# versatiles-org/versatiles-glyphs-rs

Measured on AMD Instinct MI355X. Metric: glyphs/sec (SDF raster, Noto Sans Regular full BMP set), higher is better.
Workload: dtype f64

## Files before the change

versatiles-glyphs-rs_amd/csrc/sdf_margin_kernels.hip:

```cpp
#include <hip/hip_runtime.h>
#include <stdint.h>

#include "sdf_span_support.h"

#ifndef VG_MARGIN_PART
#error "compile with -DVG_MARGIN_PART=0..6"
#endif
#define VG_MARGIN_PARTS 7
#define VG_CAT_(a, b) a##b
#define VG_CAT(a, b) VG_CAT_(a, b)

namespace vgsdf {

typedef void (*span_fn)(const GlyphDesc *, const uint2 *, uint32_t, const double *, const double *, const double *, const double *,
                        uint32_t, uint8_t *, const float4 *, const PlanHeader *);
struct MarginInstance {
	int id;
	span_fn fn;
};

#if VG_MARGIN_PART == 0
#define VG_SPAN_KERNEL sdf_margin_span_base
#include "sdf_span_kernel.inc"
__device__ unsigned long long g_span_dbg[28];
#define VG_SPAN_KERNEL sdf_margin_span_count
#define VG_SPAN_COUNTED 1
#define VG_COUNT(stmt) stmt
#include "sdf_span_kernel.inc"
#undef VG_SPAN_COUNTED
#define VG_SPAN_KERNEL sdf_margin_span_dl0
#define VG_M_DL(dl) ((void)(dl), 0.0f)
#define VG_M_E8(e, f1) ((void)(e), (void)(f1), true)
#include "sdf_span_kernel.inc"
#define VG_SPAN_KERNEL sdf_margin_span_e0
#define VG_M_E(e) ((void)(e), 0.0f)
#define VG_M_E64(e) ((void)(e), 0.0f)
#include "sdf_span_kernel.inc"
static const MarginInstance k_instances[] = {{60, sdf_margin_span_base}, {61, sdf_margin_span_count}, {62, sdf_margin_span_dl0}, {63, sdf_margin_span_e0}};

#elif VG_MARGIN_PART == 1
#define VG_SPAN_KERNEL sdf_margin_span_tkf1
#define VG_M_TK(tk, f1) ((void)(tk), (f1))
#include "sdf_span_kernel.inc"
#define VG_SPAN_KERNEL sdf_margin_span_rg0
#define VG_M_RG(r) ((void)(r), 0.0f)
#include "sdf_span_kernel.inc"
#define VG_SPAN_KERNEL sdf_margin_span_sat3
#define VG_M_SAT 3.0f
#include "sdf_span_kernel.inc"
#define VG_SPAN_KERNEL sdf_margin_span_far20
#define VG_M_FAR 20.0f
#include "sdf_span_kernel.inc"
static const MarginInstance k_instances[] = {{64, sdf_margin_span_tkf1}, {65, sdf_margin_span_rg0}, {66, sdf_margin_span_sat3}, {67, sdf_margin_span_far20}};

#elif VG_MARGIN_PART == 2
#define VG_SPAN_KERNEL sdf_margin_span_sane
#define VG_M_SANE(Mc) ((void)(Mc), true)
#include "sdf_span_kernel.inc"
#define VG_SPAN_KERNEL sdf_margin_span_bounded
#define VG_M_BOUNDED(Mc) ((void)(Mc), true)
#include "sdf_span_kernel.inc"
#define VG_SPAN_KERNEL sdf_margin_span_boxr0
#define VG_M_BOX_R(r) ((void)(r), 0.0f)
#include "sdf_span_kernel.inc"
#define VG_SPAN_KERNEL sdf_margin_span_boxband
#define VG_M_BOX_BAND(dy) ((void)(dy), true)
#include "sdf_span_kernel.inc"
static const MarginInstance k_instances[] = {{68, sdf_margin_span_sane}, {69, sdf_margin_span_bounded}, {70, sdf_margin_span_boxr0}, {71, sdf_margin_span_boxband}};

#elif VG_MARGIN_PART == 3
#define VG_SPAN_KERNEL sdf_margin_span_e64
#define VG_M_E64(e) ((void)(e), 0.0f)
#include "sdf_span_kernel.inc"
#define VG_SPAN_KERNEL sdf_margin_span_mabs0
#define VG_M_MABS0(m) ((void)(m), 0.0f)
#include "sdf_span_kernel.inc"
#define VG_SPAN_KERNEL sdf_margin_span_infl
#define VG_M_INFL 1.0f
#define VG_M_PAD(Mc) ((void)(Mc), 0.0f)
#define VG_M_GRP_SLACK 1.0f
#include "sdf_span_kernel.inc"
#define VG_SPAN_KERNEL sdf_margin_span_e_2
#define VG_M_E(e) ((e) * 0.5f)
#include "sdf_span_kernel.inc"
static const MarginInstance k_instances[] = {{72, sdf_margin_span_e64}, {73, sdf_margin_span_mabs0}, {74, sdf_margin_span_infl}, {75, sdf_margin_span_e_2}};

#elif VG_MARGIN_PART == 4
#define VG_SPAN_KERNEL sdf_margin_span_e_4
#define VG_M_E(e) ((e) * 0.25f)
#include "sdf_span_kernel.inc"
#define VG_SPAN_KERNEL sdf_margin_span_e_8
#define VG_M_E(e) ((e) * 0.125f)
#include "sdf_span_kernel.inc"
#define VG_SPAN_KERNEL sdf_margin_span_dl_2
#define VG_M_DL(dl) ((dl) * 0.5f)
#include "sdf_span_kernel.inc"
#define VG_SPAN_KERNEL sdf_margin_span_dl_4
#define VG_M_DL(dl) ((dl) * 0.25f)
#include "sdf_span_kernel.inc"
static const MarginInstance k_instances[] = {{76, sdf_margin_span_e_4}, {77, sdf_margin_span_e_8}, {78, sdf_margin_span_dl_2}, {79, sdf_margin_span_dl_4}};

#elif VG_MARGIN_PART == 5
#define VG_SPAN_KERNEL sdf_margin_span_dl_8
#define VG_M_DL(dl) ((dl) * 0.125f)
#include "sdf_span_kernel.inc"
#define VG_SPAN_KERNEL sdf_margin_span_rg_2
#define VG_M_RG(r) ((r) * 0.5f)
#include "sdf_span_kernel.inc"
#define VG_SPAN_KERNEL sdf_margin_span_rg_4
#define VG_M_RG(r) ((r) * 0.25f)
#include "sdf_span_kernel.inc"
#define VG_SPAN_KERNEL sdf_margin_span_rg_8
#define VG_M_RG(r) ((r) * 0.125f)
#include "sdf_span_kernel.inc"
static const MarginInstance k_instances[] = {{80, sdf_margin_span_dl_8}, {81, sdf_margin_span_rg_2}, {82, sdf_margin_span_rg_4}, {83, sdf_margin_span_rg_8}};
#elif VG_MARGIN_PART == 6
#define VG_SPAN_KERNEL sdf_margin_span_row_e0
#define VG_M_ROW_E(e) ((void)(e), 0.0f)
#include "sdf_span_kernel.inc"
static const MarginInstance k_instances[] = {{84, sdf_margin_span_row_e0}};

#else
#error "VG_MARGIN_PART out of range"
#endif

}

extern "C" __attribute__((visibility("hidden"))) int VG_CAT(vgsdf_margin_launch_p, VG_MARGIN_PART)(
    int kernel, uint32_t grid, uint32_t n_tiles_arg, const vgsdf::GlyphDesc *glyphs, const uint2 *tiles, const double *sx, const double *sy,
    const double *ex, const double *ey, uint32_t seg_stride, uint8_t *out, const void *boxes, hipStream_t stream)
{
	for (const vgsdf::MarginInstance &m : vgsdf::k_instances)
		if (m.id == kernel) {
			hipLaunchKernelGGL(m.fn, dim3(grid), dim3(vgsdf::TPB), 0, stream, glyphs, tiles, n_tiles_arg, sx, sy, ex, ey, seg_stride, out,
			                   (const float4 *)boxes, (const vgsdf::PlanHeader *)nullptr);
			return (int)hipGetLastError();
		}
	return -1;
}

#if VG_MARGIN_PART == 0
#define VG_MARGIN_PART_ARGS                                                                                                          \
	int kernel, uint32_t grid, uint32_t n_tiles_arg, const vgsdf::GlyphDesc *glyphs, const uint2 *tiles, const double *sx, const double *sy, \
	    const double *ex, const double *ey, uint32_t seg_stride, uint8_t *out, const void *boxes, hipStream_t stream
extern "C" int vgsdf_margin_launch_p1(VG_MARGIN_PART_ARGS);
extern "C" int vgsdf_margin_launch_p2(VG_MARGIN_PART_ARGS);
extern "C" int vgsdf_margin_launch_p3(VG_MARGIN_PART_ARGS);
extern "C" int vgsdf_margin_launch_p4(VG_MARGIN_PART_ARGS);
extern "C" int vgsdf_margin_launch_p5(VG_MARGIN_PART_ARGS);
extern "C" int vgsdf_margin_launch_p6(VG_MARGIN_PART_ARGS);

extern "C" int vgsdf_margin_known(int kernel) { return kernel >= 60 && kernel <= 84; }

extern "C" int vgsdf_margin_launch(VG_MARGIN_PART_ARGS)
{
	int (*const parts[VG_MARGIN_PARTS])(VG_MARGIN_PART_ARGS) = {vgsdf_margin_launch_p0, vgsdf_margin_launch_p1, vgsdf_margin_launch_p2,
	                                                            vgsdf_margin_launch_p3, vgsdf_margin_launch_p4, vgsdf_margin_launch_p5,
	                                                            vgsdf_margin_launch_p6};
	for (auto part : parts) {
		const int e = part(kernel, grid, n_tiles_arg, glyphs, tiles, sx, sy, ex, ey, seg_stride, out, boxes, stream);
		if (e != -1)
			return e;
	}
	return (int)hipErrorInvalidValue;
}

extern "C" int vgsdf_margin_counters(unsigned long long *out, int reset)
{
	unsigned long long h[28] = {0};
	hipError_t e = hipSuccess;
	if (out != nullptr) {
		e = hipMemcpyFromSymbol(h, HIP_SYMBOL(vgsdf::g_span_dbg), sizeof(h), 0, hipMemcpyDeviceToHost);
		static const int idx[9] = {12, 13, 14, 15, 16, 17, 20, 21, 22};
		for (int i = 0; i < 9; i++)
			out[i] = h[idx[i]];
	}
	if (e == hipSuccess && reset) {
		const unsigned long long z[28] = {0};
		e = hipMemcpyToSymbol(HIP_SYMBOL(vgsdf::g_span_dbg), z, sizeof(z), 0, hipMemcpyHostToDevice);
	}
	return (int)e;
}

extern "C" int vgsdf_margin_pair_round_counters(unsigned long long *out)
{
	unsigned long long h[28] = {0};
	const hipError_t e = hipMemcpyFromSymbol(h, HIP_SYMBOL(vgsdf::g_span_dbg), sizeof(h), 0, hipMemcpyDeviceToHost);
	for (int i = 0; i < 2; i++)
		out[i] = h[23 + i];
	return (int)e;
}

extern "C" int vgsdf_margin_stage_filter_counters(unsigned long long *out)
{
	unsigned long long h[28] = {0};
	const hipError_t e = hipMemcpyFromSymbol(h, HIP_SYMBOL(vgsdf::g_span_dbg), sizeof(h), 0, hipMemcpyDeviceToHost);
	out[0] = h[25];
	return (int)e;
}
#endif
```

versatiles-glyphs-rs_amd/csrc/sdf_span_kernel.inc:

```
#ifndef VG_POOL_MAX
#define VG_POOL_MAX 2
#endif
#ifndef VG_SPAN_KERNEL
#define VG_SPAN_KERNEL sdf_tiles_span
#endif
#ifndef VG_STAMP
#define VG_STAMP(region)
#endif
#ifndef VG_COUNT
#define VG_COUNT(stmt)
#endif
#ifndef VG_M_BOX_PADK
#define VG_M_BOX_PADK(mag) (0.02f + 2.0e-6f * (mag))
#endif
#ifndef VG_M_BOX_SAT
#define VG_M_BOX_SAT 6.2f
#endif
#ifndef VG_M_BOX_R
#define VG_M_BOX_R(r) (r)
#endif
#ifndef VG_M_BOX_BAND
#define VG_M_BOX_BAND(dy) ((dy) > 0.0f)
#endif
#ifndef VG_M_INFL
#define VG_M_INFL (1.0f + 1.0f / 512.0f)
#endif
#ifndef VG_M_GRP_SLACK
#define VG_M_GRP_SLACK 1.004f
#endif
#ifndef VG_M_PAD
#define VG_M_PAD(Mc) (0.01f + 1.0e-5f * (Mc))
#endif
#ifndef VG_M_RG
#define VG_M_RG(r) (r)
#endif
#ifndef VG_M_SAT
#define VG_M_SAT 6.2f
#endif
#ifndef VG_M_SANE
#define VG_M_SANE(Mc) ((Mc) < 1.0e6f)
#endif
#ifndef VG_M_BOUNDED
#define VG_M_BOUNDED(Mc) ((Mc) < 4096.0f)
#endif
#ifndef VG_M_MABS0
#define VG_M_MABS0(m) (m)
#endif
#ifndef VG_M_E64
#define VG_M_E64(e) (e)
#endif
#ifndef VG_M_E
#define VG_M_E(e) (e)
#endif
#ifndef VG_M_CARRY
#define VG_M_CARRY (1.0f + 1.0f / 1048576.0f)
#endif
#ifndef VG_M_DL
#define VG_M_DL(dl) (dl)
#endif
#ifndef VG_M_DL_C
#define VG_M_DL_C 17.0f
#endif
#ifndef VG_M_DL_ABS
#define VG_M_DL_ABS 3.0e-4f
#endif
#ifndef VG_M_E8
#define VG_M_E8(e, f1) (8.0f * (e) <= (f1))
#endif
#ifndef VG_M_FAR
#define VG_M_FAR 35.9f
#endif
#ifndef VG_M_TK_PUSH
#define VG_M_TK_PUSH(tk) ((tk) * 1.001f + 1e-30f)
#endif
#ifndef VG_M_TK
#define VG_M_TK(tk, f1) (tk)
#endif
#ifndef VG_M_ROW_E
#define VG_M_ROW_E(e) (e)
#endif

__global__ __launch_bounds__(TPB, 4) void VG_SPAN_KERNEL(const GlyphDesc *__restrict__ glyphs,
                                                          const uint2 *__restrict__ tiles, uint32_t n_tiles,
                                                          const double *__restrict__ seg_sx,
                                                          const double *__restrict__ seg_sy,
                                                          const double *__restrict__ seg_ex,
                                                          const double *__restrict__ seg_ey, uint32_t seg_stride,
                                                          uint8_t *__restrict__ out, const float4 *__restrict__ boxes,
                                                          const PlanHeader *__restrict__ plan)
{
	if (plan != nullptr && (!plan->ok || blockIdx.x >= plan->n_main))
		return;
#ifdef VG_SPAN_STAMPED
	unsigned long long st_acc[12] = {0, 0, 0, 0, 0, 0, 0, 0, 0, 0, 0, 0}, st_last = 0;
#endif
#if defined(VG_SPAN_STAMPED) || defined(VG_SPAN_COUNTED)
	unsigned long long cn_pairs = 0, cn_rounds = 0, cn_tc = 0, cn_fb = 0, cn_fbl = 0;
	unsigned long long cn_over = 0, cn_fb_pool = 0, cn_fb_lane = 0;
	unsigned long long cn_half = 0, cn_leave = 0;
	unsigned long long cn_row_fb = 0;
#endif
	VG_STAMP(-1);
	constexpr uint32_t GRP = 8, NGRP = FCHUNK / GRP;
	static_assert(NGRP == 32 && TPB == FCHUNK, "one candidate bit per group, one staging thread per record");
	__shared__ __attribute__((aligned(16))) float s_rec[5][FCHUNK];
	__shared__ double e_pt[4][FCHUNK];
	float *const s_vx = s_rec[0], *const s_vy = s_rec[1], *const s_dx = s_rec[2], *const s_dy = s_rec[3], *const s_inv = s_rec[4];
	double *const e_vx = e_pt[0], *const e_vy = e_pt[1], *const e_wx = e_pt[2], *const e_wy = e_pt[3];
	__shared__ int s_delta[DELTA_CAP];
	__shared__ uint32_t s_mbits[2];
	__shared__ __attribute__((aligned(16))) float s_g[3][NGRP];
	__shared__ float st_ub2[SPAN_TILES * TPB];
	__shared__ uint16_t st_byte[SPAN_TILES * TPB];
	__shared__ uint32_t st_pix[SPAN_TILES * TPB];
	constexpr uint32_t QCAP = 256;
	__shared__ uint32_t q_pair[TPB / 64][QCAP];
	__shared__ uint32_t q_min[TPB / 64][64];

	const uint32_t tid = threadIdx.x, lane = threadIdx.x & 63;
	const uint32_t wv = (uint32_t)__builtin_amdgcn_readfirstlane((int)(threadIdx.x >> 6));
	const uint32_t rot = wave_rot(blockIdx.x);
	const uint32_t pw = ((wv + rot) & 3u) * 64u;
	const uint32_t tile = xcd_remap(blockIdx.x, n_tiles);
	const uint2 t = tiles[tile];
	const GlyphDesc g = glyphs[t.x];
	const uint32_t npix = g.w * g.h;
	const uint32_t p0 = t.y & ~255u, T = min(max(t.y & 255u, 1u), SPAN_TILES);
	const uint32_t p_end = min(p0 + T * (uint32_t)TPB, npix);

	const uint32_t r_first = p0 / g.w, r_last = (p_end - 1) / g.w;
	const int y_hi = (int)(g.h - 1 - r_first), y_lo = (int)(g.h - 1 - r_last);
	const uint32_t stride = (g.w + 1) | 1u;
	const uint32_t n_delta = (r_last - r_first + 1) * stride;
	for (uint32_t i = tid; i < n_delta; i += TPB)
		s_delta[i] = 0;
	const float wh = (float)max(g.w, g.h);
	const int hw = (int)(g.w >> 1), hh = (int)(g.h >> 1);
	for (uint32_t k = 0; k < T; k++) {
		st_ub2[k * TPB + tid] = __builtin_inff();
		st_byte[k * TPB + tid] = 0x00FFu;
		const uint32_t oc = min(p0 + k * TPB + pw + lane, npix - 1);
		const uint32_t row = oc / g.w;
		st_pix[k * TPB + tid] = pix_pack((float)((int)(oc - row * g.w) - hw) + 0.5f, row - r_first);
	}
	int y_mid = y_hi - hh;
	asm volatile("" : "+s"(y_mid));
	const float mpix = 0.5f * wh + 1.0f;
	uint32_t par = 0;
	if (tid == 0)
		s_mbits[0] = __float_as_uint(mpix);
	const float mabs0 = VG_M_MABS0(fmaxf(fmaxf(fabsf((float)g.x0), fabsf((float)g.y0)),
	                                     fmaxf(fabsf((float)g.x0 + (float)g.w), fabsf((float)g.y0 + (float)g.h))));

	const bool use_boxes = boxes != nullptr && g.n_seg > 2 * FCHUNK;
	for (uint32_t c0 = 0; c0 < g.n_seg; c0 += FCHUNK) {
		const uint32_t cnt = min((uint32_t)FCHUNK, g.n_seg - c0);
		VG_STAMP(0);
		__syncthreads();
		VG_STAMP(1);
		if (use_boxes) {
			const float4 bb = boxes[chunk_box_index(g.seg_off, t.x, c0 / FCHUNK)];
			const float mag = fmaxf(fmaxf(fabsf(bb.x), fabsf(bb.y)), fmaxf(fmaxf(fabsf(bb.z), fabsf(bb.w)), wh));
			const float padk = VG_M_BOX_PADK(mag);
			const float ry0 = (float)y_lo + 0.5f, ry1 = (float)y_hi + 0.5f;
			const float dy = fmaxf(bb.y - ry1, ry0 - bb.w) - padk;
			float dx = fmaxf(bb.x - ((float)g.w - 0.5f), 0.5f - bb.z) - padk;
			dx = dx > 0.0f ? dx : 0.0f;
			const float R = VG_M_BOX_R(VG_M_BOX_SAT + padk);
			if (VG_M_BOX_BAND(dy) && __builtin_fmaf(dy, dy, dx * dx) > R * R)
				continue;
		}
		constexpr float INFL = VG_M_INFL;
		{
			int gx0 = g.x0, gy0 = g.y0;
			asm volatile("" : "+s"(gx0), "+s"(gy0));
			const double ox = (double)gx0 + (double)hw, oy = (double)gy0 + (double)hh;
			const uint32_t i = tid;
			float mf = 0.0f;
			float fvx = 1.0e18f, fvy = 1.0e18f, fdx = 0.0f, fdy = 0.0f, finv = 0.0f;
			uint32_t nrow = 0;
			int ya = 0;
			bool row_exact = false;
			if (i < cnt) {
				const size_t s = (size_t)(g.seg_off + c0 + i) * seg_stride;
				const double vx = seg_sx[s], vy = seg_sy[s], wx = seg_ex[s], wy = seg_ey[s];
				e_vx[i] = vx;
				e_vy[i] = vy;
				e_wx[i] = wx;
				e_wy[i] = wy;
				const double dx = wx - vx, dy = wy - vy;
				const double l2 = dx * dx + dy * dy;
				fvx = (float)(vx - ox);
				fvy = (float)(vy - oy);
				fdx = (float)dx;
				fdy = (float)dy;
				finv = (l2 > 1e-20 && l2 < 1e30) ? __builtin_amdgcn_rcpf((float)l2) : 0.0f;
				mf = fmaxf(fmaxf(fabsf(fvx), fabsf(fvy)), fmaxf(fabsf(fvx + fdx), fabsf(fvy + fdy))) * 1.00001f;
				mf = mf >= 0.0f ? mf : __builtin_inff();
				const float tv = fvy - 0.5f, tw = (fvy + fdy) - 0.5f;
				const float e_row = VG_M_ROW_E(__builtin_fmaf(STAGE_ROW_C, fmaxf(mf, mpix), STAGE_ROW_ABS));
				const bool decided = __builtin_fminf(int_dist(tv), int_dist(tw)) > e_row && mf < STAGE_M_MAX;
				const int cv = (int)__builtin_ceilf(tv), cw = (int)__builtin_ceilf(tw);
				const int c_lo = y_lo - hh, c_hi = y_hi + 1 - hh;
				const int ca = min(max(min(cv, cw), c_lo), c_hi), cb = min(max(max(cv, cw), c_lo), c_hi);
				ya = ca + hh;
				nrow = decided ? (uint32_t)(cb - ca) : 0u;
				row_exact = vy != wy && !decided;
			}
			const bool row_fb = __builtin_amdgcn_ballot_w64(row_exact) != 0;
			VG_COUNT(cn_row_fb += row_fb);
			if (row_fb && row_exact) {
				const double vy = e_vy[i], wy = e_wy[i];
				const double y0c = (double)gy0 + 0.5;
				const double band_lo = (double)y_lo + y0c, band_hi = (double)y_hi + y0c;
				const bool up = vy < wy;
				const double lo = up ? vy : wy, hi = up ? wy : vy;
				if (hi > band_lo && lo <= band_hi) {
					ya = first_ge(lo, y0c, y_lo, y_hi + 1);
					const int yb = first_ge(hi, y0c, y_lo, y_hi + 1);
					nrow = yb > ya ? (uint32_t)(yb - ya) : 0u;
				}
			}
			s_vx[i] = fvx;
			s_vy[i] = fvy;
			s_dx[i] = fdx;
			s_dy[i] = fdy;
			s_inv[i] = finv;
			const uint32_t mb = wave_max_u32(__float_as_uint(mf));
			if (lane == 0)
				atomicMax(&s_mbits[par], mb);

			{
				const uint32_t gb = tid & ~(GRP - 1);
				const uint32_t ai = min(gb + GRP / 2, cnt - 1);
				const float ax = __shfl(fvx, (int)(ai & 63u)), ay = __shfl(fvy, (int)(ai & 63u));
				float r2 = 0.0f;
				if (i < cnt) {
					const float wx = fvx + fdx, wy = fvy + fdy;
					const float ex = fvx - ax, ey = fvy - ay, fx = wx - ax, fy = wy - ay;
					const float dv = __builtin_fmaf(ey, ey, ex * ex), dw = __builtin_fmaf(fy, fy, fx * fx);
					r2 = dv > dw ? dv : dw;
				}
				r2 = __uint_as_float(oct_max_u32(__float_as_uint(r2)));
				if ((tid & (GRP - 1)) == 0) {
					const bool empty = gb >= cnt;
					s_g[0][tid / GRP] = empty ? 1.0e18f : ax;
					s_g[1][tid / GRP] = empty ? 1.0e18f : ay;
					s_g[2][tid / GRP] = empty ? 0.0f : __builtin_amdgcn_sqrtf(r2) * (INFL * INFL * VG_M_GRP_SLACK);
				}
			}

			{
				const uint32_t incl = wave_scan_add(nrow);
				const uint32_t total = (uint32_t)__builtin_amdgcn_readlane((int)incl, 63);
				auto cross = [&](double vx, double vy, double dx, double dy, bool up, int yy) {
					const double x0c = (double)gx0 + 0.5, y0c = (double)gy0 + 0.5;
					const double pyy = (double)yy + y0c;
					const double tc = (pyy - vy) / dy;
					const double xc = vx + tc * dx;
					const int k = first_ge(xc, x0c, 0, (int)g.w);
					if (k < (int)g.w)
						atomicAdd(&s_delta[(uint32_t)(y_hi - yy) * stride + (uint32_t)k], up ? -1 : 1);
				};
				if (total != 0 && total <= QCAP) {
					uint32_t off = incl - nrow;
#pragma unroll 1
					for (uint32_t r = 0; r < nrow; r++)
						q_pair[wv][off++] = (lane << 10) | (uint32_t)(y_hi - (ya + (int)r));
					__builtin_amdgcn_fence(__ATOMIC_RELEASE, "wavefront");
					__builtin_amdgcn_wave_barrier();
					for (uint32_t base = 0; base < total; base += 64) {
						const uint32_t idx = base + lane;
						if (idx < total) {
							const uint32_t e = q_pair[wv][idx];
							const uint32_t si = (tid & ~63u) + (e >> 10);
							const double vx = e_vx[si], vy = e_vy[si], wx = e_wx[si], wy = e_wy[si];
							cross(vx, vy, wx - vx, wy - vy, vy < wy, y_hi - (int)(e & 1023u));
						}
					}
					__builtin_amdgcn_fence(__ATOMIC_ACQ_REL, "wavefront");
					__builtin_amdgcn_wave_barrier();
				} else if (total != 0) {
					if (nrow != 0) {
						const double vx = e_vx[i], vy = e_vy[i], wx = e_wx[i], wy = e_wy[i];
						for (uint32_t r = 0; r < nrow; r++)
							cross(vx, vy, wx - vx, wy - vy, vy < wy, ya + (int)r);
					}
				}
			}
		}
		VG_STAMP(2);
		__syncthreads();
		VG_STAMP(3);
		const float Mc = __uint_as_float(s_mbits[par]);
		par ^= 1u;
		if (tid == 0)
			s_mbits[par] = __float_as_uint(mpix);
		const bool sane = VG_M_SANE(Mc);
		const bool bounded = VG_M_BOUNDED(Mc);
		const float pad = VG_M_PAD(Mc);
		const uint32_t n_groups = (cnt + GRP - 1) / GRP;

		const float4 *q_vx = reinterpret_cast<const float4 *>(s_vx), *q_vy = reinterpret_cast<const float4 *>(s_vy);
		const float4 *q_dx = reinterpret_cast<const float4 *>(s_dx), *q_dy = reinterpret_cast<const float4 *>(s_dy);
		const float4 *q_inv = reinterpret_cast<const float4 *>(s_inv);
		const float M = Mc;
		const float e64 = VG_M_E64(VG_E64_C * M * (M + mabs0 + M));
		const float herr_c1 = VG_HERR_SLACK * VG_HERR_C1 * M, herr_c3 = VG_HERR_SLACK * VG_HERR_C3 * M * M + e64;

#pragma unroll 1
		for (uint32_t k = 0; k < T; k++) {
			asm volatile("" ::: "memory");
			const uint32_t o = p0 + k * TPB + pw + lane;
			if (p0 + k * TPB + pw >= npix)
				continue;
			const uint32_t pe = st_pix[k * TPB + tid];
			const float rpx = pix_rpx(pe);
			const int roff = (int)pix_roff(pe);
			const float rpy = (float)(y_mid - roff) + 0.5f;
			float ub2 = st_ub2[k * TPB + tid];
			VG_STAMP(0);


			uint32_t cand = n_groups >= 32 ? 0xFFFFFFFFu : ((1u << n_groups) - 1u);
			if (bounded) {
				uint32_t D2p[NGRP / 2];
				uint32_t dmin = __float_as_uint(ub2);
				const float4 *gx4 = reinterpret_cast<const float4 *>(s_g[0]), *gy4 = reinterpret_cast<const float4 *>(s_g[1]);
				const float4 *gr4 = reinterpret_cast<const float4 *>(s_g[2]);
				auto near4 = [&](uint32_t b, const float4 ax, const float4 ay) {
					const float axs[4] = {ax.x, ax.y, ax.z, ax.w}, ays[4] = {ay.x, ay.y, ay.z, ay.w};
					uint32_t d2[4];
#pragma unroll
					for (int j = 0; j < 4; j++) {
						const float ddx = rpx - axs[j], ddy = rpy - ays[j];
						d2[j] = __float_as_uint(__builtin_fmaf(ddy, ddy, ddx * ddx));
					}
					asm("v_min3_u32 %0, %1, %2, %3" : "=v"(dmin) : "v"(dmin), "v"(d2[0]), "v"(d2[1]));
					asm("v_min3_u32 %0, %1, %2, %3" : "=v"(dmin) : "v"(dmin), "v"(d2[2]), "v"(d2[3]));
					D2p[b * 2] = __builtin_amdgcn_perm(d2[1], d2[0], 0x07060302u);
					D2p[b * 2 + 1] = __builtin_amdgcn_perm(d2[3], d2[2], 0x07060302u);
				};
				if (n_groups == NGRP) {
#pragma unroll
					for (uint32_t b = 0; b < NGRP / 4; b++)
						near4(b, gx4[b], gy4[b]);
				} else {
					float4 ax = gx4[0], ay = gy4[0];
#pragma unroll
					for (uint32_t b = 0; b < NGRP / 4; b++) {
						if (b * 4 < n_groups) {
							if (b + 1 == NGRP / 4) {
								near4(b, ax, ay);
								break;
							}
							const float4 nx = gx4[b + 1], ny = gy4[b + 1];
							near4(b, ax, ay);
							asm volatile("" ::"v"(nx.x), "v"(nx.y), "v"(nx.z), "v"(nx.w), "v"(ny.x), "v"(ny.y), "v"(ny.z), "v"(ny.w));
							ax = nx;
							ay = ny;
						} else {
							break;
						}
					}
				}
				ub2 = __uint_as_float(dmin);
				float U = (__builtin_amdgcn_sqrtf(ub2) * INFL + pad) * INFL;
				U = U < VG_M_SAT ? U : VG_M_SAT;
				const float Ui = (U + pad * INFL) * VG_M_GRP_SLACK;
				uint32_t rej;
				asm volatile("" : "=v"(rej));
				auto reject4 = [&](uint32_t b) {
					const float4 r = gr4[b];
					const float rs[4] = {r.x, r.y, r.z, r.w};
#pragma unroll
					for (int j = 3; j >= 0; j--) {
						const uint32_t pk = D2p[b * 2 + j / 2];
						const float d2 = __uint_as_float((j & 1) ? pk : (pk << 16));
						const float tt = Ui + VG_M_RG(rs[j]);
						const float diff = __builtin_fmaf(tt, tt, -d2);
						rej = __builtin_amdgcn_alignbit(rej, __float_as_uint(diff), 31);
					}
				};
				static_assert(NGRP / 4 == 8, "one case per block of four groups");
				if (n_groups == NGRP) {
#pragma unroll
					for (int b = NGRP / 4 - 1; b >= 0; b--)
						reject4((uint32_t)b);
				} else switch ((n_groups + 3) / 4) {
				default: reject4(7); [[fallthrough]];
				case 7: reject4(6); [[fallthrough]];
				case 6: reject4(5); [[fallthrough]];
				case 5: reject4(4); [[fallthrough]];
				case 4: reject4(3); [[fallthrough]];
				case 3: reject4(2); [[fallthrough]];
				case 2: reject4(1); [[fallthrough]];
				case 1: reject4(0);
				}
				cand &= ~rej;
			}

			VG_STAMP(6);
			uint32_t k1 = 0xFFFFFFFFu;
			auto rec4 = [](const float4 *row, uint32_t goff, uint32_t hq) {
				return *reinterpret_cast<const float4 *>(reinterpret_cast<const char *>(row) + goff + 16u * hq);
			};
			auto half_min = [&](uint32_t acc, uint32_t goff, uint32_t hq, float qx, float qy) {
				const float4 vx4 = rec4(q_vx, goff, hq), vy4 = rec4(q_vy, goff, hq), dx4 = rec4(q_dx, goff, hq), dy4 = rec4(q_dy, goff, hq),
				             iv4 = rec4(q_inv, goff, hq);
				const uint32_t f0 = __float_as_uint(sc_filter(qx, qy, vx4.x, vy4.x, dx4.x, dy4.x, iv4.x));
				const uint32_t f1 = __float_as_uint(sc_filter(qx, qy, vx4.y, vy4.y, dx4.y, dy4.y, iv4.y));
				const uint32_t f2 = __float_as_uint(sc_filter(qx, qy, vx4.z, vy4.z, dx4.z, dy4.z, iv4.z));
				const uint32_t f3 = __float_as_uint(sc_filter(qx, qy, vx4.w, vy4.w, dx4.w, dy4.w, iv4.w));
				uint32_t mn;
				asm("v_min3_u32 %0, %1, %2, %3" : "=v"(mn) : "v"(acc), "v"(f0), "v"(f1));
				asm("v_min3_u32 %0, %1, %2, %3" : "=v"(acc) : "v"(mn), "v"(f2), "v"(f3));
				return acc;
			};
			auto group_min = [&](uint32_t acc, uint32_t goff, float qx, float qy) {
				acc = half_min(acc, goff, 0, qx, qy);
				__builtin_amdgcn_sched_barrier(0);
				return half_min(acc, goff, 1, qx, qy);
			};
			if (sane) {
				if (o >= npix)
					cand = 0;
				const uint32_t c = (uint32_t)__builtin_popcount(cand);
				const uint32_t incl = wave_scan_add(c);
				const uint32_t total = (uint32_t)__builtin_amdgcn_readlane((int)incl, 63);
				VG_COUNT(cn_pairs += total; cn_rounds += (total + 63) / 64; cn_tc += 1);
				if (total == 0) {
					st_ub2[k * TPB + tid] = ub2;
					VG_COUNT(cn_leave += 1);
					continue;
				}
				if (total <= QCAP) {
					uint32_t *qp = &q_pair[wv][incl - c];
					q_min[wv][lane] = 0xFFFFFFFFu;
					uint32_t m = cand;
					while (m) {
						*qp = (lane << 18) | ((uint32_t)__builtin_ctz(m) << 5);
						__builtin_amdgcn_sched_barrier(0);
						qp++;
						m &= m - 1;
					}
					__builtin_amdgcn_fence(__ATOMIC_RELEASE, "wavefront");
					__builtin_amdgcn_wave_barrier();
					const uint32_t tail = ((total - 1u) & 63u) + 1u;
					const uint32_t lim = tail <= 32u ? total - tail : total;
					uint32_t e = q_pair[wv][min(lane, total - 1)];
					const uint32_t lim64 = lim + 64;
					for (uint32_t next = 64; next < lim64; next += 64) {
						const uint32_t idx_next = next + lane;
						const uint32_t e_next = q_pair[wv][min(idx_next, total - 1)];
						const uint32_t src4 = e >> 16;
						const float qx = __uint_as_float((uint32_t)__builtin_amdgcn_ds_bpermute((int)src4, (int)__float_as_uint(rpx)));
						const float qy = __uint_as_float((uint32_t)__builtin_amdgcn_ds_bpermute((int)src4, (int)__float_as_uint(rpy)));
						const uint32_t mn = group_min(0xFFFFFFFFu, e & 0xFFFFu, qx, qy);
						if (idx_next < lim64)
							atomicMin(reinterpret_cast<uint32_t *>(reinterpret_cast<char *>(q_min[wv]) + src4), mn);
						e = e_next;
					}
					if (lim != total) {
						VG_COUNT(cn_half += 1);
						const uint32_t eh = __builtin_amdgcn_permlane32_swap(e, e, false, false)[0];
						const uint32_t src4 = eh >> 16;
						const float qx = __uint_as_float((uint32_t)__builtin_amdgcn_ds_bpermute((int)src4, (int)__float_as_uint(rpx)));
						const float qy = __uint_as_float((uint32_t)__builtin_amdgcn_ds_bpermute((int)src4, (int)__float_as_uint(rpy)));
						const uint32_t mn = half_min(0xFFFFFFFFu, eh & 0xFFFFu, lane >> 5, qx, qy);
						if ((lane & 31u) < tail)
							atomicMin(reinterpret_cast<uint32_t *>(reinterpret_cast<char *>(q_min[wv]) + src4), mn);
					}
					__builtin_amdgcn_fence(__ATOMIC_ACQ_REL, "wavefront");
					__builtin_amdgcn_wave_barrier();
					k1 = q_min[wv][lane];
				} else {
					VG_COUNT(cn_over += 1);
					uint32_t m = cand;
					while (m) {
						const uint32_t gq = (uint32_t)__builtin_ctz(m);
						m &= m - 1;
						k1 = group_min(k1, gq * 32u, rpx, rpy);
					}
				}
			}

			VG_STAMP(7);
			bool have = false;
			uint32_t b_in = 255u, b_out = 0u;
			double best = __builtin_huge_val();
			auto exact_at = [&](double qpx, double qpy, uint32_t i) {
				const double vx = e_vx[i], vy = e_vy[i], wx = e_wx[i], wy = e_wy[i];
				const double dx = wx - vx, dy = wy - vy;
				return exact_dist_sq(qpx, qpy, vx, vy, wx, wy, dx, dy, dx * dx + dy * dy);
			};
			bool undecided = false;
			float Tk = __builtin_inff();
			if (!sane) {
				int gx0 = g.x0, gy0 = g.y0;
				asm volatile("" : "+s"(gx0), "+s"(gy0));
				const double px = (double)pix_col(rpx, hw) + ((double)gx0 + 0.5), py = (double)(y_hi - roff) + ((double)gy0 + 0.5);
				for (uint32_t j = 0; j < cnt; j++) {
					const double d2 = exact_at(px, py, j);
					best = d2 < best ? d2 : best;
				}
				have = true;
			} else if (k1 != 0xFFFFFFFFu) {
				const float f1 = __uint_as_float(k1);
				const float sq = __builtin_amdgcn_sqrtf(f1);
				const float e = VG_M_E(__builtin_fmaf(herr_c1, sq, __builtin_fmaf(VG_HERR_C2S, f1, herr_c3)));
				float U = f1 + e;
				const float uf = U * VG_M_CARRY;
				ub2 = uf < ub2 ? uf : ub2;
				const float s = __builtin_fmaf(32.0f, sq, 0.5f);
				const float dl = VG_M_DL(__builtin_fmaf(VG_M_DL_C * e, __builtin_amdgcn_rcpf(sq), VG_M_DL_ABS));
				const float fr = __builtin_amdgcn_fractf(s);
				const float mn = fr < 1.0f - fr ? fr : 1.0f - fr;
				const bool far = f1 - e > VG_M_FAR;
				const bool decided = far || (VG_M_E8(e, f1) && mn > dl);
				if (decided) {
					const int q = far ? 200 : (int)s;
					b_in = (uint32_t)min(191 + q, 255);
					b_out = (uint32_t)max(191 - q, 0);
				} else {
					if (!(U >= 0.0f))
						U = __builtin_inff();
					Tk = U + e64;
					for (int it = 0; it < 3; it++)
						Tk = U + e64 + VG_M_E(filter_err(Tk, M));
					Tk = VG_M_TK_PUSH(Tk);
					if (!(Tk - VG_M_E(filter_err(Tk, M)) - e64 > U))
						Tk = __builtin_inff();
					Tk = VG_M_TK(Tk, f1);
					undecided = true;
				}
			}
			VG_STAMP(8);
			{
				unsigned long long amb = __ballot(undecided);
				VG_COUNT(cn_fb += amb != 0; cn_fbl += (unsigned long long)__builtin_popcountll(amb);
				         cn_fb_pool += amb != 0 && VG_POOL_MAX != 0 && (uint32_t)__builtin_popcountll(amb) <= (uint32_t)VG_POOL_MAX;
				         cn_fb_lane += amb != 0 && !(VG_POOL_MAX != 0 && (uint32_t)__builtin_popcountll(amb) <= (uint32_t)VG_POOL_MAX));
				if (VG_POOL_MAX != 0 && (uint32_t)__builtin_popcountll(amb) <= (uint32_t)VG_POOL_MAX) {
					while (amb) {
						const int src = (int)__builtin_ctzll(amb);
						amb &= amb - 1;
						const float spx = __uint_as_float((uint32_t)__builtin_amdgcn_readlane((int)__float_as_uint(rpx), src));
						const float spy = __uint_as_float((uint32_t)__builtin_amdgcn_readlane((int)__float_as_uint(rpy), src));
						const float sTk = __uint_as_float((uint32_t)__builtin_amdgcn_readlane((int)__float_as_uint(Tk), src));
						int gx0 = g.x0, gy0 = g.y0;
						asm volatile("" : "+s"(gx0), "+s"(gy0));
						const double dpx = (double)pix_col(spx, hw) + ((double)gx0 + 0.5);
						const double dpy = (double)(y_hi - __builtin_amdgcn_readlane(roff, src)) + ((double)gy0 + 0.5);
						uint32_t scand = (uint32_t)__builtin_amdgcn_readlane((int)cand, src);
						double wbest = __builtin_huge_val();
						while (scand) {
							uint32_t sel = scand;
							for (uint32_t i = lane >> 3; i != 0; i--)
								sel &= sel - 1;
							if (sel != 0) {
								const uint32_t j = (uint32_t)__builtin_ctz(sel) * GRP + (lane & 7u);
								if (j < cnt && !(sc_filter(spx, spy, s_vx[j], s_vy[j], s_dx[j], s_dy[j], s_inv[j]) > sTk)) {
									const double d2 = exact_at(dpx, dpy, j);
									wbest = d2 < wbest ? d2 : wbest;
								}
							}
#pragma unroll
							for (uint32_t i = 0; i < 8; i++)
								scand &= scand - 1;
						}
						wbest = wave_min_f64(wbest);
						if ((int)lane == src)
							best = wbest;
					}
				} else if (undecided) {
					int gx0 = g.x0, gy0 = g.y0;
					asm volatile("" : "+s"(gx0), "+s"(gy0));
					const double px = (double)pix_col(rpx, hw) + ((double)gx0 + 0.5), py = (double)(y_hi - roff) + ((double)gy0 + 0.5);
					uint32_t m = cand;
					while (m) {
						const uint32_t gq = (uint32_t)__builtin_ctz(m);
						m &= m - 1;
						uint32_t hit = 0;
#pragma unroll 1
						for (uint32_t hq = 0; hq < 2; hq++) {
							const float4 vx4 = q_vx[2 * gq + hq], vy4 = q_vy[2 * gq + hq], dx4 = q_dx[2 * gq + hq], dy4 = q_dy[2 * gq + hq],
							             iv4 = q_inv[2 * gq + hq];
							hit |= !(sc_filter(rpx, rpy, vx4.x, vy4.x, dx4.x, dy4.x, iv4.x) > Tk) ? (1u << (4 * hq)) : 0u;
							hit |= !(sc_filter(rpx, rpy, vx4.y, vy4.y, dx4.y, dy4.y, iv4.y) > Tk) ? (2u << (4 * hq)) : 0u;
							hit |= !(sc_filter(rpx, rpy, vx4.z, vy4.z, dx4.z, dy4.z, iv4.z) > Tk) ? (4u << (4 * hq)) : 0u;
							hit |= !(sc_filter(rpx, rpy, vx4.w, vy4.w, dx4.w, dy4.w, iv4.w) > Tk) ? (8u << (4 * hq)) : 0u;
						}
						while (hit) {
							const uint32_t j = gq * GRP + (uint32_t)__builtin_ctz(hit);
							hit &= hit - 1;
							if (j < cnt) {
								const double d2 = exact_at(px, py, j);
								best = d2 < best ? d2 : best;
							}
						}
					}
				}
				have = have || undecided;
			}
			VG_STAMP(9);
			if (have) {
				b_in = quantise(best, true);
				b_out = quantise(best, false);
			}
			const uint32_t old = st_byte[k * TPB + tid];
			b_in = min(b_in, old & 255u);
			b_out = max(b_out, old >> 8);
			st_byte[k * TPB + tid] = (uint16_t)(b_in | (b_out << 8));
			st_ub2[k * TPB + tid] = ub2;
			VG_STAMP(10);
		}
	}

	__syncthreads();
	{
		const uint32_t n_rows = r_last - r_first + 1;
		for (uint32_t r = tid; r < n_rows; r += TPB) {
			int *drow = s_delta + r * stride;
			int acc = 0;
#pragma unroll 4
			for (uint32_t c = 0; c < g.w; c++) {
				acc += drow[c];
				drow[c] = acc;
			}
		}
	}
	__syncthreads();
	for (uint32_t k = 0; k < T; k++) {
		const uint32_t o = p0 + k * TPB + pw + lane;
		if (o < npix) {
			const uint32_t pe = st_pix[k * TPB + tid];
			const int wn = s_delta[pix_roff(pe) * stride + (uint32_t)pix_col(pix_rpx(pe), hw)];
			const uint32_t sb = st_byte[k * TPB + tid];
			out[g.out_off + o] = (uint8_t)(wn != 0 ? (sb & 255u) : (sb >> 8));
		}
	}
	VG_STAMP(11);
#if defined(VG_SPAN_STAMPED) || defined(VG_SPAN_COUNTED)
	if (lane == 0) {
#ifdef VG_SPAN_STAMPED
		for (int r = 0; r < 12; r++)
			atomicAdd(&g_span_dbg[r], st_acc[r]);
#endif
		atomicAdd(&g_span_dbg[12], 1ull);
		atomicAdd(&g_span_dbg[13], cn_pairs);
		atomicAdd(&g_span_dbg[14], cn_rounds);
		atomicAdd(&g_span_dbg[15], cn_tc);
		atomicAdd(&g_span_dbg[16], cn_fb);
		atomicAdd(&g_span_dbg[17], cn_fbl);
		atomicAdd(&g_span_dbg[20], cn_over);
		atomicAdd(&g_span_dbg[21], cn_fb_pool);
		atomicAdd(&g_span_dbg[22], cn_fb_lane);
		atomicAdd(&g_span_dbg[23], cn_half);
		atomicAdd(&g_span_dbg[24], cn_leave);
		atomicAdd(&g_span_dbg[25], cn_row_fb);
	}
#endif
}

#undef VG_SPAN_KERNEL
#undef VG_STAMP
#undef VG_COUNT
#undef VG_M_BOX_PADK
#undef VG_M_BOX_SAT
#undef VG_M_BOX_R
#undef VG_M_BOX_BAND
#undef VG_M_INFL
#undef VG_M_GRP_SLACK
#undef VG_M_PAD
#undef VG_M_RG
#undef VG_M_SAT
#undef VG_M_SANE
#undef VG_M_BOUNDED
#undef VG_M_MABS0
#undef VG_M_E64
#undef VG_M_E
#undef VG_M_CARRY
#undef VG_M_DL
#undef VG_M_DL_C
#undef VG_M_DL_ABS
#undef VG_M_E8
#undef VG_M_FAR
#undef VG_M_TK_PUSH
#undef VG_M_TK
#undef VG_M_ROW_E
```

Measured before the change: 47.47 million.

## Add shared-memory work queue for pixel sweeps and pooled edge crossings

Replaces the static per-wave pixel-chunk assignment in the span kernel with a dynamic shared-memory work queue. Waves claim 64-pixel units with an atomic counter. Edge row crossings are deferred into a block-wide shared buffer, and the first wave to take queue slot 0 processes them alongside the next sweep instead of each wave handling its own. The aim is to even out load imbalance between waves and overlap crossing work with distance evaluation. In exchange it adds shared-memory atomics, a CAS reservation loop and extra LDS, and both paths are enabled by default.

```diff
diff --git a/versatiles-glyphs-rs_amd/csrc/sdf_margin_kernels.hip b/versatiles-glyphs-rs_amd/csrc/sdf_margin_kernels.hip
--- a/versatiles-glyphs-rs_amd/csrc/sdf_margin_kernels.hip
+++ b/versatiles-glyphs-rs_amd/csrc/sdf_margin_kernels.hip
@@ -198,4 +198,12 @@
 	out[0] = h[25];
 	return (int)e;
 }
+
+extern "C" int vgsdf_margin_queue_counters(unsigned long long *out)
+{
+	unsigned long long h[28] = {0};
+	const hipError_t e = hipMemcpyFromSymbol(h, HIP_SYMBOL(vgsdf::g_span_dbg), sizeof(h), 0, hipMemcpyDeviceToHost);
+	out[0] = h[26];
+	return (int)e;
+}
 #endif
diff --git a/versatiles-glyphs-rs_amd/csrc/sdf_span_kernel.inc b/versatiles-glyphs-rs_amd/csrc/sdf_span_kernel.inc
--- a/versatiles-glyphs-rs_amd/csrc/sdf_span_kernel.inc
+++ b/versatiles-glyphs-rs_amd/csrc/sdf_span_kernel.inc
@@ -1,5 +1,11 @@
 #ifndef VG_POOL_MAX
 #define VG_POOL_MAX 2
+#endif
+#ifndef VG_QUEUE_SWEEPS
+#define VG_QUEUE_SWEEPS 1
+#endif
+#ifndef VG_QUEUE_CROSS
+#define VG_QUEUE_CROSS 1
 #endif
 #ifndef VG_SPAN_KERNEL
 #define VG_SPAN_KERNEL sdf_tiles_span
@@ -99,6 +105,7 @@
 	unsigned long long cn_over = 0, cn_fb_pool = 0, cn_fb_lane = 0;
 	unsigned long long cn_half = 0, cn_leave = 0;
 	unsigned long long cn_row_fb = 0;
+	unsigned long long cn_cross = 0;
 #endif
 	VG_STAMP(-1);
 	constexpr uint32_t GRP = 8, NGRP = FCHUNK / GRP;
@@ -116,11 +123,25 @@
 	constexpr uint32_t QCAP = 256;
 	__shared__ uint32_t q_pair[TPB / 64][QCAP];
 	__shared__ uint32_t q_min[TPB / 64][64];
+#if VG_QUEUE_SWEEPS || VG_QUEUE_CROSS
+	__shared__ uint32_t s_queue[2][2];
+#endif
+#if VG_QUEUE_CROSS
+	constexpr uint32_t CCAP = 768;
+	__shared__ uint32_t s_cross[CCAP];
+	constexpr uint32_t Q_FIRST = 1;
+#else
+	constexpr uint32_t Q_FIRST = 0;
+#endif
 
 	const uint32_t tid = threadIdx.x, lane = threadIdx.x & 63;
 	const uint32_t wv = (uint32_t)__builtin_amdgcn_readfirstlane((int)(threadIdx.x >> 6));
+#if VG_QUEUE_SWEEPS
+	const uint32_t pw = wv * 64u;
+#else
 	const uint32_t rot = wave_rot(blockIdx.x);
 	const uint32_t pw = ((wv + rot) & 3u) * 64u;
+#endif
 	const uint32_t tile = xcd_remap(blockIdx.x, n_tiles);
 	const uint2 t = tiles[tile];
 	const GlyphDesc g = glyphs[t.x];
@@ -147,8 +168,33 @@
 	asm volatile("" : "+s"(y_mid));
 	const float mpix = 0.5f * wh + 1.0f;
 	uint32_t par = 0;
-	if (tid == 0)
+	if (tid == 0) {
 		s_mbits[0] = __float_as_uint(mpix);
+#if VG_QUEUE_SWEEPS || VG_QUEUE_CROSS
+		s_queue[0][0] = Q_FIRST;
+		s_queue[0][1] = 0;
+#endif
+	}
+#if VG_QUEUE_SWEEPS || VG_QUEUE_CROSS
+	auto take = [&](uint32_t slot) {
+		uint32_t u = 0;
+		if (lane == 0)
+			u = atomicAdd(&s_queue[slot][0], 1u);
+		return (uint32_t)__builtin_amdgcn_readfirstlane((int)u);
+	};
+#endif
+#if VG_QUEUE_SWEEPS
+	const uint32_t n_units = (p_end - p0 + 63u) / 64u;
+#endif
+	auto cross = [&](int gx0, int gy0, double vx, double vy, double dx, double dy, bool up, int yy) {
+		const double x0c = (double)gx0 + 0.5, y0c = (double)gy0 + 0.5;
+		const double pyy = (double)yy + y0c;
+		const double tc = (pyy - vy) / dy;
+		const double xc = vx + tc * dx;
+		const int k = first_ge(xc, x0c, 0, (int)g.w);
+		if (k < (int)g.w)
+			atomicAdd(&s_delta[(uint32_t)(y_hi - yy) * stride + (uint32_t)k], up ? -1 : 1);
+	};
 	const float mabs0 = VG_M_MABS0(fmaxf(fmaxf(fabsf((float)g.x0), fabsf((float)g.y0)),
 	                                     fmaxf(fabsf((float)g.x0 + (float)g.w), fabsf((float)g.y0 + (float)g.h))));
 
@@ -253,16 +299,32 @@
 			{
 				const uint32_t incl = wave_scan_add(nrow);
 				const uint32_t total = (uint32_t)__builtin_amdgcn_readlane((int)incl, 63);
-				auto cross = [&](double vx, double vy, double dx, double dy, bool up, int yy) {
-					const double x0c = (double)gx0 + 0.5, y0c = (double)gy0 + 0.5;
-					const double pyy = (double)yy + y0c;
-					const double tc = (pyy - vy) / dy;
-					const double xc = vx + tc * dx;
-					const int k = first_ge(xc, x0c, 0, (int)g.w);
-					if (k < (int)g.w)
-						atomicAdd(&s_delta[(uint32_t)(y_hi - yy) * stride + (uint32_t)k], up ? -1 : 1);
-				};
+#if VG_QUEUE_CROSS
+				uint32_t cbase = CCAP;
+				if (total != 0) {
+					if (lane == 0) {
+						uint32_t seen = s_queue[par][1];
+						while (seen + total <= CCAP) {
+							const uint32_t was = atomicCAS(&s_queue[par][1], seen, seen + total);
+							if (was == seen) {
+								cbase = seen;
+								s_queue[par][0] = 0;
+								break;
+							}
+							seen = was;
+						}
+					}
+					cbase = (uint32_t)__builtin_amdgcn_readfirstlane((int)cbase);
+				}
+				if (cbase != CCAP) {
+					uint32_t off = cbase + incl - nrow;
+#pragma unroll 1
+					for (uint32_t r = 0; r < nrow; r++)
+						s_cross[off++] = (tid << 10) | (uint32_t)(y_hi - (ya + (int)r));
+				} else
+#endif
 				if (total != 0 && total <= QCAP) {
+					VG_COUNT(cn_cross += (total + 63) / 64);
 					uint32_t off = incl - nrow;
 #pragma unroll 1
 					for (uint32_t r = 0; r < nrow; r++)
@@ -275,16 +337,17 @@
 							const uint32_t e = q_pair[wv][idx];
 							const uint32_t si = (tid & ~63u) + (e >> 10);
 							const double vx = e_vx[si], vy = e_vy[si], wx = e_wx[si], wy = e_wy[si];
-							cross(vx, vy, wx - vx, wy - vy, vy < wy, y_hi - (int)(e & 1023u));
+							cross(gx0, gy0, vx, vy, wx - vx, wy - vy, vy < wy, y_hi - (int)(e & 1023u));
 						}
 					}
 					__builtin_amdgcn_fence(__ATOMIC_ACQ_REL, "wavefront");
 					__builtin_amdgcn_wave_barrier();
 				} else if (total != 0) {
+					VG_COUNT(cn_cross += 1);
 					if (nrow != 0) {
 						const double vx = e_vx[i], vy = e_vy[i], wx = e_wx[i], wy = e_wy[i];
 						for (uint32_t r = 0; r < nrow; r++)
-							cross(vx, vy, wx - vx, wy - vy, vy < wy, ya + (int)r);
+							cross(gx0, gy0, vx, vy, wx - vx, wy - vy, vy < wy, ya + (int)r);
 					}
 				}
 			}
@@ -293,9 +356,17 @@
 		__syncthreads();
 		VG_STAMP(3);
 		const float Mc = __uint_as_float(s_mbits[par]);
+#if VG_QUEUE_SWEEPS || VG_QUEUE_CROSS
+		const uint32_t qs = par;
+#endif
 		par ^= 1u;
-		if (tid == 0)
+		if (tid == 0) {
 			s_mbits[par] = __float_as_uint(mpix);
+#if VG_QUEUE_SWEEPS || VG_QUEUE_CROSS
+			s_queue[par][0] = Q_FIRST;
+			s_queue[par][1] = 0;
+#endif
+		}
 		const bool sane = VG_M_SANE(Mc);
 		const bool bounded = VG_M_BOUNDED(Mc);
 		const float pad = VG_M_PAD(Mc);
@@ -308,17 +379,57 @@
 		const float e64 = VG_M_E64(VG_E64_C * M * (M + mabs0 + M));
 		const float herr_c1 = VG_HERR_SLACK * VG_HERR_C1 * M, herr_c3 = VG_HERR_SLACK * VG_HERR_C3 * M * M + e64;
 
+#if VG_QUEUE_CROSS
+		auto pooled_crossings = [&]() {
+			int gx0 = g.x0, gy0 = g.y0;
+			asm volatile("" : "+s"(gx0), "+s"(gy0));
+			const uint32_t n_cross = (uint32_t)__builtin_amdgcn_readfirstlane((int)s_queue[qs][1]);
+			VG_COUNT(cn_cross += (n_cross + 63) / 64);
+			for (uint32_t base = 0; base < n_cross; base += 64) {
+				const uint32_t idx = base + lane;
+				if (idx < n_cross) {
+					const uint32_t e = s_cross[idx];
+					const uint32_t si = e >> 10;
+					const double vx = e_vx[si], vy = e_vy[si], wx = e_wx[si], wy = e_wy[si];
+					cross(gx0, gy0, vx, vy, wx - vx, wy - vy, vy < wy, y_hi - (int)(e & 1023u));
+				}
+			}
+		};
+#endif
+#if VG_QUEUE_SWEEPS
+#pragma unroll 1
+		for (;;) {
+			asm volatile("" ::: "memory");
+			uint32_t u = take(qs);
+#if VG_QUEUE_CROSS
+			if (u == 0) {
+				pooled_crossings();
+				continue;
+			}
+			u -= 1u;
+#endif
+			if (u >= n_units)
+				break;
+			const uint32_t sidx = u * 64u + lane;
+			const uint32_t o = p0 + sidx;
+#else
+#if VG_QUEUE_CROSS
+		if (take(qs) == 0)
+			pooled_crossings();
+#endif
 #pragma unroll 1
 		for (uint32_t k = 0; k < T; k++) {
 			asm volatile("" ::: "memory");
+			const uint32_t sidx = k * TPB + tid;
 			const uint32_t o = p0 + k * TPB + pw + lane;
 			if (p0 + k * TPB + pw >= npix)
 				continue;
-			const uint32_t pe = st_pix[k * TPB + tid];
+#endif
+			const uint32_t pe = st_pix[sidx];
 			const float rpx = pix_rpx(pe);
 			const int roff = (int)pix_roff(pe);
 			const float rpy = (float)(y_mid - roff) + 0.5f;
-			float ub2 = st_ub2[k * TPB + tid];
+			float ub2 = st_ub2[sidx];
 			VG_STAMP(0);
 
 
@@ -430,7 +541,7 @@
 				const uint32_t total = (uint32_t)__builtin_amdgcn_readlane((int)incl, 63);
 				VG_COUNT(cn_pairs += total; cn_rounds += (total + 63) / 64; cn_tc += 1);
 				if (total == 0) {
-					st_ub2[k * TPB + tid] = ub2;
+					st_ub2[sidx] = ub2;
 					VG_COUNT(cn_leave += 1);
 					continue;
 				}
@@ -608,11 +719,11 @@
 				b_in = quantise(best, true);
 				b_out = quantise(best, false);
 			}
-			const uint32_t old = st_byte[k * TPB + tid];
+			const uint32_t old = st_byte[sidx];
 			b_in = min(b_in, old & 255u);
 			b_out = max(b_out, old >> 8);
-			st_byte[k * TPB + tid] = (uint16_t)(b_in | (b_out << 8));
-			st_ub2[k * TPB + tid] = ub2;
+			st_byte[sidx] = (uint16_t)(b_in | (b_out << 8));
+			st_ub2[sidx] = ub2;
 			VG_STAMP(10);
 		}
 	}
@@ -659,6 +770,7 @@
 		atomicAdd(&g_span_dbg[23], cn_half);
 		atomicAdd(&g_span_dbg[24], cn_leave);
 		atomicAdd(&g_span_dbg[25], cn_row_fb);
+		atomicAdd(&g_span_dbg[26], cn_cross);
 	}
 #endif
 }
```

Result: slower. 43.69 million (-8.0%).
